# vivansxu/rafiki

Hardware: AMD Instinct MI355X
Metric: images/sec aggregate over concurrent VGG-small 32x32x3 HPO trials (1 trial/GPU) (higher is better)
Workload: dtype fp32; 1 GPU; model=VGG-small 32x32x3 (8 conv3x3+BN+ReLU, 4 maxpool, FC512, FC10), global_batch=256, per_trial_batch=256, parallelism=single trial, 1 GPU, optimizer=SGD nesterov momentum + wd (fused flat-arena kernel), hipgraph=True

## Files before the change

### csrc/kernels/bnf.hip

```cpp
#include "common.h"
#include <algorithm>
#include <cstdint>

namespace {

RK_DEV int rk_log2_dev(int v) { return (v > 0 && (v & (v - 1)) == 0) ? 31 - __builtin_clz(v) : -1; }

RK_DEV int idiv(int a, int d, int log2d) { return log2d >= 0 ? a >> log2d : a / d; }

RK_DEV float act_f(float z, int act, float slope) {
  return act == 1 ? fmaxf(z, 0.f) : act == 2 ? (z > 0.f ? z : z * slope) : z;
}
RK_DEV float act_d(float z, int act, float slope) {
  return act == 1 ? (z > 0.f ? 1.f : 0.f) : act == 2 ? (z > 0.f ? 1.f : slope) : 1.f;
}

template <bool POOL>
__global__ __launch_bounds__(256) void bnf_fwd_kernel(const float* __restrict__ y, const double* __restrict__ slots,
                                                      int SL, double count, const float* __restrict__ gamma,
                                                      const float* __restrict__ beta, float eps, float* rmean,
                                                      float* rvar, float mom, const float* __restrict__ scale_in,
                                                      const float* __restrict__ shift_in, float* __restrict__ coeffs,
                                                      float* __restrict__ out, int Nb, int H, int W, int C, int act,
                                                      float slope) {
  extern __shared__ float s_dyn[];
  float* s_sc = s_dyn;
  float* s_sh = s_dyn + C;
  for (int c = threadIdx.x; c < C; c += 256) {
    float sc, sh;
    if (slots) {
      double s = 0.0, ss = 0.0;
      for (int l = 0; l < SL; ++l) {
        s += slots[(long long)l * 2 * C + c];
        ss += slots[(long long)l * 2 * C + C + c];
      }
      const double mean = s / count;
      const double var = fmax(ss / count - mean * mean, 0.0);
      const double rstd = 1.0 / sqrt(var + (double)eps);
      sc = (float)((double)gamma[c] * rstd);
      sh = (float)((double)beta[c] - mean * (double)gamma[c] * rstd);
      if (blockIdx.x == 0) {
        coeffs[c] = (float)mean;
        coeffs[C + c] = (float)rstd;
        coeffs[2 * C + c] = sc;
        coeffs[3 * C + c] = sh;
        if (rmean) {
          rmean[c] = (float)((1.0 - mom) * rmean[c] + mom * mean);
          rvar[c] = (float)((1.0 - mom) * rvar[c] + mom * var * count / fmax(count - 1.0, 1.0));
        }
      }
    } else {
      sc = scale_in[c];
      sh = shift_in[c];
    }
    s_sc[c] = sc;
    s_sh[c] = sh;
  }
  if (!out) return;
  __syncthreads();
  const int G = C >> 2;
  const int Ho = POOL ? H >> 1 : H, Wo = POOL ? W >> 1 : W;
  const int lG = rk_log2_dev(G), lWo = rk_log2_dev(Wo), lHo = rk_log2_dev(Ho);
  const int total = Nb * Ho * Wo * G;
  for (int i = blockIdx.x * 256 + threadIdx.x; i < total; i += gridDim.x * 256) {
    const int pix = idiv(i, G, lG);
// ... 532 lines not shown
```

### csrc/kernels/winograd4.hip

```cpp
#include <type_traits>
#include "common.h"
#include <cstdlib>

namespace {

#include "wino_wt.h"

constexpr int KC = 8;
enum { WF_RELU = 1, WF_BIAS = 2, WF_STATS = 4, WF_LRELU = 8, WF_BNB = 512, WF_BNP = 1024, WF_POOL = 2048 };
constexpr int WF_POOLED = WF_BIAS | WF_RELU | WF_POOL;

typedef __attribute__((ext_vector_type(2))) float f32x2;

struct W4Params {
  const float* x;
  const float* u;
  float* y;
  const float* bias;
  double* stats;
  const float* gate;
  int Nb, H, W, C, N;
  int TW, THW, ntiles, ncb, slotMask, flags;
  unsigned long long xbytes, ubytes, ybytes;
  int bpg;
  long long gx, gu, gy, gbias;
  const float* pro;
};

constexpr unsigned OOB = 0x80000000u;
constexpr int W4_PRO_MAXC = 512;

RK_DEV int swz(int row) { return ((row >> 2) & 3) << 1; }
RK_DEV int swzw(int row) { return (((row >> 2) & 1) << 1) | (((row >> 3) & 1) << 2) | ((row >> 4) & 1); }
RK_DEV int swzp(int row) { return swzw(row) & 6; }

RK_DEV __amdgpu_buffer_rsrc_t rsrc(const float* base, unsigned long long bytes) {
  return __builtin_amdgcn_make_buffer_rsrc(const_cast<float*>(base), (short)0, (int)(unsigned)bytes, 0x00020000);
}

RK_DEV void bt6(float d0, float d1, float d2, float d3, float d4, float d5, float (&t)[6]) {
  t[0] = 4.f * d0 - 5.f * d2 + d4;
// ... 55 lines not shown
  constexpr int NT = 64 * WM * WN;
  constexpr int T = 16 * WM;
  constexpr int BNC = 16 * WN;
  constexpr int IT = T * KC / NT;
  constexpr int UL = P * BNC * 4 / NT;
  constexpr int UNITS = P * BNC * KC / 4;
  constexpr int UBL = (UNITS + NT - 1) / NT;
  constexpr int ULR = UB ? 1 : UL, UBR = UB ? UBL : 1;
  static_assert(IT >= 1 && IT * NT == T * KC && UL * NT == P * BNC * 4, "tile shape");
  static_assert(!UB || (MO == 4 && BNC == 32), "blocked weights: F(4x4), 32-channel output blocks");
  static_assert(!WS || (NS == 2 && UB), "warp-specialised: two stages, blocked weights");
  __shared__ __attribute__((aligned(16))) float Vs[NS][P][T][KC];
  __shared__ __attribute__((aligned(16))) float Us[NS][P][BNC][KC];
  __shared__ float Ps[PRO ? 2 * W4_PRO_MAXC : 1];
  if constexpr (PRO) {
    for (int i = threadIdx.x; i < 2 * p.C; i += (int)blockDim.x)
      Ps[i < p.C ? i : W4_PRO_MAXC + i - p.C] = p.pro[i];
    __syncthreads();
  }
  const int lane = threadIdx.x & 63, wave = threadIdx.x >> 6;
  const bool compute = !WS || wave < WM * WN;
  const int tid = (WS && !compute) ? (int)threadIdx.x - NT : (int)threadIdx.x;
  const int wm = wave % WM, wn = (wave / WM) % WN;
  const int b0 = xcd_remap(blockIdx.x, gridDim.x);
  const int grp = b0 / p.bpg, b = b0 - grp * p.bpg;
  const int cb = b % p.ncb, tb = b / p.ncb;
  const int tbase = tb * T, cbase = cb * BNC;
  const float* const gxp = p.x + grp * p.gx;
  const float* const gup = p.u + grp * p.gu;
  float* const gyp = p.y + grp * p.gy;
  const float* const gbp = p.bias ? p.bias + grp * p.gbias : nullptr;

// ... 875 lines not shown
                                   const long long* meta, void* stream) {
  if (nblocks <= 0) return RK_OK;
  hipLaunchKernelGGL(wt_all_kernel, dim3(nblocks), dim3(256), 0, (hipStream_t)stream, arena, dst, (const int4*)desc,
                     meta);
  RK_LAUNCH_CHECK();
  return RK_OK;
}

namespace {
struct GfwdArgs {
  const float* x; const float* u; float* y; const float* bias; double* stats; int slotMask; const float* gate;
  int Nb, H, W, C, N, flags, groups;
  long long gx, gu, gy, gbias;
  const float* pro;
  void* stream;
};

template <int MO, int WM, int WN, int MINW, int NS = 1, bool UB = false, bool WS = false, bool PRO = false>
int launch_gfwd(const GfwdArgs& a) {
  constexpr int T = 16 * WM, BNC = 16 * WN, P = (MO + 2) * (MO + 2);
  const int Nb = a.Nb, H = a.H, W = a.W, C = a.C, N = a.N, flags = a.flags, groups = a.groups;
  if (Nb <= 0 || H <= 0 || W <= 0 || (H % MO) || (W % MO) || C <= 0 || (C % KC) || N <= 0 || groups <= 0)
    return RK_EBADARG;
  if ((flags & (WF_STATS | WF_BNB | WF_BNP)) && !a.stats) return RK_EBADARG;
  if ((flags & (WF_BNB | WF_BNP)) && (!a.gate || !a.bias)) return RK_EBADARG;
  if ((flags & WF_BIAS) && !a.bias) return RK_EBADARG;
  if (groups > 1 && (flags & (WF_STATS | WF_BNB | WF_BNP))) return RK_EUNSUPPORTED;
  if (PRO != (a.pro != nullptr)) return RK_EBADARG;
  if ((flags & WF_POOL) && (flags != WF_POOLED || PRO || (H & 1) || (W & 1))) return RK_EUNSUPPORTED;
  if (PRO && (groups > 1 || (flags & ~WF_STATS) || C > W4_PRO_MAXC)) return RK_EUNSUPPORTED;
  W4Params p;
  p.x = a.x; p.u = a.u; p.y = a.y; p.bias = a.bias; p.stats = a.stats; p.gate = a.gate;
  p.pro = a.pro;
  p.Nb = Nb; p.H = H; p.W = W; p.C = C; p.N = N;
  p.TW = W / MO;
  p.THW = (H / MO) * (W / MO);
  const long long nt = (long long)Nb * p.THW;
  if (nt >= (1LL << 30)) return RK_EBADARG;
  p.ntiles = (int)nt;
  p.ncb = rk_cdiv(N, BNC);
  p.xbytes = 4ull * Nb * H * W * C;
  p.ubytes = UB ? 4ull * P * rk_cdiv(N, 32) * 32 * C : 4ull * P * N * C;
  p.ybytes = (flags & WF_POOL) ? 4ull * Nb * (H / 2) * (W / 2) * N : 4ull * Nb * H * W * N;
  const unsigned long long gbytes = (flags & WF_BNP) ? 4 * p.ybytes : p.ybytes;
  if (p.xbytes >= 0x7fffffffull || p.ubytes >= 0x7fffffffull || gbytes >= 0x7fffffffull) return RK_EUNSUPPORTED;
  p.slotMask = a.slotMask;
  p.flags = flags;
  p.gx = a.gx; p.gu = a.gu; p.gy = a.gy; p.gbias = a.gbias;
// ... 57 lines not shown

template <int NR>
int gfwd_dispatch(const GfwdRow (&rows)[NR], int variant, const GfwdArgs& a) {
  for (const GfwdRow& r : rows)
    if (r.variant == variant && r.pro == (a.pro != nullptr)) return r.launch(a);
  return a.pro ? RK_EUNSUPPORTED : RK_EBADARG;
}
}

extern "C" int rk_wino4_conv_grp(const float* x, const float* u, float* y, const float* bias, double* stats,
                                 int slotMask, const float* gate, int Nb, int H, int W, int C, int N, int flags,
                                 int variant, int groups, long long gx, long long gu, long long gy, long long gbias,
                                 const float* pro, void* stream) {
  return gfwd_dispatch(W4_ROWS, variant, {x, u, y, bias, stats, slotMask, gate, Nb, H, W, C, N, flags, groups, gx, gu,
                                          gy, gbias, pro, stream});
}

extern "C" int rk_wino2s_conv_grp(const float* x, const float* u, float* y, const float* bias, double* stats,
                                  int slotMask, const float* gate, int Nb, int H, int W, int C, int N, int flags,
                                  int variant, int groups, long long gx, long long gu, long long gy, long long gbias,
                                  void* stream) {
  return gfwd_dispatch(W2S_ROWS, variant, {x, u, y, bias, stats, slotMask, gate, Nb, H, W, C, N, flags, groups, gx,
                                           gu, gy, gbias, nullptr, stream});
}

extern "C" int rk_wino4_wgrad(const float* dy, const float* x, float* out, int Nb, int H, int W, int Co, int Ci,
                              int splits, int accumulate, int variant, const float* xpro, void* stream) {
  if (Nb <= 0 || H <= 0 || W <= 0 || (H & 3) || (W & 3) || Co <= 0 || Ci <= 0 || splits <= 0) return RK_EBADARG;
  if (splits > 1 && accumulate) return RK_EBADARG;
  if (variant < 0 || variant > 2) return RK_EBADARG;
// ... 60 lines not shown
    }
#pragma unroll
    for (int a = 0; a < 6; ++a) {
      float o[6];
      a6(mm[a][0], mm[a][1], mm[a][2], mm[a][3], o);
#pragma unroll
      for (int b = 0; b < 6; ++b) res[a * 6 + b][e] = o[b];
    }
  }
  float* dst = m + t * C + 4 * c4;
  const int ps = T * C;
#pragma unroll
  for (int q = 0; q < 36; ++q) *(f32x4*)(dst + q * ps) = res[q];
}

template <bool PL = false, int VW = 4>
__global__ __launch_bounds__(256) void w4pt_x_kernel(const float* __restrict__ x, void* __restrict__ v, int H,
                                                     int W, int C, int TW, int THW, int total4, int T,
                                                     const float* __restrict__ pro) {
  typedef __attribute__((ext_vector_type(VW))) float fvec;
  typedef __attribute__((ext_vector_type(VW))) __bf16 bvec;
  const int i = blockIdx.x * 256 + threadIdx.x;
  if (i >= total4) return;
  const int CV = C / VW;
  const int cv = i % CV, t = i / CV;
  const int n = t / THW, r = t - n * THW, ty = r / TW;
  const int oy = 4 * ty - 1, ox = 4 * (r - ty * TW) - 1;
  fvec psc, psh;
#pragma unroll
  for (int e = 0; e < VW; ++e) psc[e] = 1.f, psh[e] = 0.f;
  if (pro) {
    psc = *(const fvec*)(pro + VW * cv);
    psh = *(const fvec*)(pro + C + VW * cv);
  }
  fvec d[36];
#pragma unroll
  for (int a = 0; a < 6; ++a)
#pragma unroll
    for (int b = 0; b < 6; ++b) {
      const int yy = oy + a, xx = ox + b;
      const bool in = (unsigned)yy < (unsigned)H && (unsigned)xx < (unsigned)W;
      fvec val;
      if (in) {
        val = *(const fvec*)(x + ((n * H + yy) * W + xx) * C + VW * cv);
      } else {
#pragma unroll
        for (int e = 0; e < VW; ++e) val[e] = 0.f;
      }
      if (pro && in) {
#pragma unroll
        for (int e = 0; e < VW; ++e) val[e] = fmaxf(fmaf(val[e], psc[e], psh[e]), 0.f);
      }
      d[a * 6 + b] = val;
    }
#pragma unroll
  for (int b = 0; b < 6; ++b)
#pragma unroll
    for (int e = 0; e < VW; ++e) {
      float o[6];
      bt6(d[b][e], d[6 + b][e], d[12 + b][e], d[18 + b][e], d[24 + b][e], d[30 + b][e], o);
#pragma unroll
      for (int a = 0; a < 6; ++a) d[a * 6 + b][e] = o[a];
    }
  const int ps = T * C;
// ... 247 lines not shown

}

extern "C" int rk_wino4_pt_transform(const float* dy, const float* x, float* m, float* v, int Nb, int H, int W,
                                     int Co, int Ci, const float* xpro, void* stream) {
  if (Nb <= 0 || H <= 0 || W <= 0 || (H & 3) || (W & 3) || Co <= 0 || Ci <= 0) return RK_EBADARG;
  if ((Co & 3) || (Ci & 3)) return RK_EUNSUPPORTED;
  const int TW = W / 4, THW = (H / 4) * (W / 4);
  const long long T = (long long)Nb * THW;
  if (36 * T * Co >= (1ll << 31) || 36 * T * Ci >= (1ll << 31)) return RK_EUNSUPPORTED;
  const long long ty = T * Co / 4, tx = T * Ci / 4;
  hipLaunchKernelGGL(w4pt_dy_kernel, dim3((unsigned)((ty + 255) / 256)), dim3(256), 0, (hipStream_t)stream, dy, m, H,
                     W, Co, TW, THW, (int)ty, (int)T);
  RK_LAUNCH_CHECK();
  hipLaunchKernelGGL(w4pt_x_kernel<false>, dim3((unsigned)((tx + 255) / 256)), dim3(256), 0, (hipStream_t)stream, x,
                     v, H, W, Ci, TW, THW, (int)tx, (int)T, xpro);
  RK_LAUNCH_CHECK();
  return RK_OK;
}

extern "C" int rk_wino4_pt_output(const float* du, float* out, int Co, int Ci, int accumulate, int nslab,
                                  long long slab, void* stream) {
  if (Co <= 0 || Ci <= 0 || nslab <= 0 || (nslab > 1 && slab < 36ll * Co * Ci)) return RK_EBADARG;
  if ((Ci & 3) || 36ll * Co * Ci >= (1ll << 31)) return RK_EUNSUPPORTED;
  const long long g2 = (long long)Co * Ci / 2;
  hipLaunchKernelGGL(w4pt_out_kernel, dim3((unsigned)((g2 + 255) / 256)), dim3(256), 0, (hipStream_t)stream, du,
                     out, Co, Ci, accumulate, nslab, slab);
  RK_LAUNCH_CHECK();
  return RK_OK;
}

// ... 234 lines not shown
    if (vw == 4)
      hipLaunchKernelGGL(w4pt_conv_outv_kernel<4>, dim3((unsigned)blocksv), dim3(64), 0, (hipStream_t)stream, yt, y,
                         bias, stats, slotMask, gate, Nb, H, W, N, TW, THW, (int)T, flags, nslab, slab, qs, ts, slope);
    else
      hipLaunchKernelGGL(w4pt_conv_outv_kernel<2>, dim3((unsigned)blocksv), dim3(64), 0, (hipStream_t)stream, yt, y,
                         bias, stats, slotMask, gate, Nb, H, W, N, TW, THW, (int)T, flags, nslab, slab, qs, ts, slope);
    RK_LAUNCH_CHECK();
    return RK_OK;
  }
  hipLaunchKernelGGL(w4pt_conv_out_kernel, dim3((unsigned)blocks), dim3(256), 0, (hipStream_t)stream, yt, y, bias,
                     stats, slotMask, gate, Nb, H, W, N, TW, THW, (int)T, flags, nslab, slab, qs, ts, slope);
  RK_LAUNCH_CHECK();
  return RK_OK;
}

extern "C" int rk_wino4_pt_input(const float* x, float* v, int Nb, int H, int W, int C, const float* pro,
                                 void* stream) {
  if (Nb <= 0 || H <= 0 || W <= 0 || (H & 3) || (W & 3) || C <= 0) return RK_EBADARG;
  if (C & 3) return RK_EUNSUPPORTED;
  const int TW = W / 4, THW = (H / 4) * (W / 4);
  const long long T = (long long)Nb * THW;
  if (36 * T * C >= (1ll << 31)) return RK_EUNSUPPORTED;
  const long long tx = T * C / 4;
  hipLaunchKernelGGL(w4pt_x_kernel<false>, dim3((unsigned)((tx + 255) / 256)), dim3(256), 0, (hipStream_t)stream, x,
                     v, H, W, C, TW, THW, (int)tx, (int)T, pro);
  RK_LAUNCH_CHECK();
  return RK_OK;
}

extern "C" int rk_x6p_w4_input(const float* x, void* v, int Nb, int H, int W, int C, const float* pro,
                               void* stream) {
  if (Nb <= 0 || H <= 0 || W <= 0 || (H & 3) || (W & 3) || C <= 0) return RK_EBADARG;
  if (C & 3) return RK_EUNSUPPORTED;
  const int TW = W / 4, THW = (H / 4) * (W / 4);
  const long long T = (long long)Nb * THW;
  if (108 * T * C >= (1ll << 31) || (long long)Nb * H * W * C >= (1ll << 31)) return RK_EUNSUPPORTED;
  static const int vw = [] {
    const char* e = std::getenv("RAFIKI_PT_X_VW");
    return e && std::atoi(e) == 2 ? 2 : 4;
  }();
  const long long tx = T * C / vw;
  if (vw == 4)
    hipLaunchKernelGGL((w4pt_x_kernel<true, 4>), dim3((unsigned)((tx + 255) / 256)), dim3(256), 0,
                       (hipStream_t)stream, x, v, H, W, C, TW, THW, (int)tx, (int)T, pro);
  else
    hipLaunchKernelGGL((w4pt_x_kernel<true, 2>), dim3((unsigned)((tx + 255) / 256)), dim3(256), 0,
                       (hipStream_t)stream, x, v, H, W, C, TW, THW, (int)tx, (int)T, pro);
  RK_LAUNCH_CHECK();
  return RK_OK;
}

extern "C" int rk_x6p_w4_wgrad_transform(const float* dy, const float* x, void* mt, void* vt, int Nb, int H, int W,
                                         int Co, int Ci, void* stream) {
  if (Nb <= 0 || H <= 0 || W <= 0 || (H & 3) || (W & 3) || Co <= 0 || Ci <= 0) return RK_EBADARG;
  if ((Co & 3) || (Ci & 3)) return RK_EUNSUPPORTED;
  const int TW = W / 4, THW = (H / 4) * (W / 4);
  const long long T = (long long)Nb * THW;
  if (108 * T * Co >= (1ll << 31) || 108 * T * Ci >= (1ll << 31)) return RK_EUNSUPPORTED;
  if ((long long)Nb * H * W * (Co > Ci ? Co : Ci) >= (1ll << 31)) return RK_EUNSUPPORTED;
  if (T % 32 == 0 && Co % 8 == 0 && Ci % 8 == 0) {
    hipLaunchKernelGGL(w4pt_planesT_kernel<true>, dim3((unsigned)(T / 32), Co / 8), dim3(64), 0, (hipStream_t)stream,
                       dy, (bf16*)mt, H, W, Co, TW, THW, (int)T);
    RK_LAUNCH_CHECK();
    hipLaunchKernelGGL(w4pt_planesT_kernel<false>, dim3((unsigned)(T / 32), Ci / 8), dim3(64), 0, (hipStream_t)stream,
// ... 14 lines not shown
```

### rafiki_amd/engine/convnet.py

```python
from __future__ import annotations

import math
import os
import warnings
from typing import List, Optional, Sequence

import numpy as np
import torch
import torch.nn.functional as TF

from ..ops import f32 as S
from ..ops import functional as F
from ..ops.graphs import capture as _capture, device_sync as _device_sync
from .flat import FlatAdam, FlatParams, FlatSGD, check_clip_norm, init_const, init_kaiming

VGG_SMALL_CFG = (64, 64, 'M', 128, 128, 'M', 256, 256, 'M', 512, 512, 'M')
DTYPES = ('fp32', 'bf16')


def default_dtype() -> str:
    d = os.environ.get('RAFIKI_DTYPE', 'fp32').lower()
    d = {'float32': 'fp32', 'f32': 'fp32', 'bfloat16': 'bf16'}.get(d, d)
    if d not in DTYPES:
        raise ValueError('RAFIKI_DTYPE must be one of {}'.format(DTYPES))
# ... 361 lines not shown
        nxt = self.blocks[bi + 1]
        return (not pool and nxt[1] == cout and nxt[4] == hw and ww.lazy('u4b', bi + 1) is not None
                and S.bn_on_load_ok(B, hw, hw, cout, nxt[2]))

    def _fwd_bwd_gpu_f32(self, x, labels):
        fl = self.flat
        B = x.shape[0]
        accs = self._bn_accumulators()
        if not self._acc_zeroed_by_prologue:
            self._bn_acc_flat.zero_()
        ww = self._wino_train()
        if ww is not None:
            ww.refresh()
        acts, saved, h = [x], [], x
        pros, hpro = [None], None
        for bi, (name, cin, cout, pool, hw) in enumerate(self.blocks):
            wk = ww.conv_sets(bi) if ww is not None else {}
            if not self.bn:
                c = self._block_coeffs(bi)
                y = S.conv_fwd(h, fl.w(name + '.w'), bias=fl.w(name + '.b'),
                               act=F.ACT_NONE if pool else F.ACT_RELU, **wk)
                h = S.bn_eval(y, c[2], c[3], pool=True, act=F.ACT_RELU) if pool else y
                saved.append((y, c))
                acts.append(h)
                continue
            rm, rv = self.running_stats(bi)
            y = S.conv_fwd(h, fl.w(name + '.w'), stats_acc=accs[bi][0], pro=hpro, **wk)
            if self._bn_on_load(bi, B, ww):
                coeffs = S.bn_finalize(y, accs[bi][0], B * hw * hw, fl.w(name + '.gamma'), fl.w(name + '.beta'),
                                       self.bn_eps, rm, rv, self.bn_momentum)
                h, hpro = y, coeffs
            else:
                h, coeffs = S.bn_fwd(y, accs[bi][0], B * hw * hw, fl.w(name + '.gamma'), fl.w(name + '.beta'),
                                     self.bn_eps, rm, rv, self.bn_momentum, pool=pool, act=F.ACT_RELU)
                hpro = None
            saved.append((y, coeffs))
            acts.append(h)
            pros.append(hpro)
        in_saved = None
        if self.input_bn:
            raw = h.reshape(B, 1, 1, self.feat_dim)
            acc_f, acc_b = accs[-1]
            S.col_stats(raw.view(B, self.feat_dim), acc_f)
            rm, rv = self.running_stats('in')
            h, coeffs = S.bn_fwd(raw, acc_f, B, fl.w('in_bn.gamma'), fl.w('in_bn.beta'), self.bn_eps, rm, rv,
                                 self.bn_momentum, pool=False, act=F.ACT_NONE)
            in_saved = (raw, coeffs)
        feat = h.reshape(B, self.feat_dim)
        if self.feature_dropout > 0.0:
            self._drop(feat, -1, self.feature_dropout, forward=True)
# ... 740 lines not shown
```

### rafiki_amd/ops/_lib.py

```python
from __future__ import annotations

import ctypes as C
import os
import threading
from pathlib import Path

_NATIVE = Path(__file__).resolve().parent.parent / "_native"
KERNEL_LIB = Path(os.environ["RAFIKI_KERNEL_LIB"]) if os.environ.get("RAFIKI_KERNEL_LIB") else \
    _NATIVE / "librafiki_kernels.so"

_lock = threading.Lock()
_lib = None

vp, i32, i64, f32, f64 = C.c_void_p, C.c_int, C.c_longlong, C.c_float, C.c_double
u32p = C.POINTER(C.c_uint)

_SIGS = {
    "rk_igemm": [i32, i32, i32, vp, vp, vp, vp, vp, vp, i32, i32, i32, i32, i32, i32, i32, i32, i32, i32,
                 i32, i32, i64, i32, f32, f32, i64, i64, vp],
    "rk_hconv": [i32, i32, vp, vp, vp, vp, vp, vp, i32, i32, i32, i32, i32, i32, i32, i32, f32, f32, i64, i64, i32,
                 vp],
    "rk_hconv_wgrad": [vp, vp, vp, i32, i32, i32, i32, i32, i32, i64, i64, vp],
    "rk_bn_bwd_reduce_acc": [vp, vp, vp, vp, vp, i32, i32, i32, i32, i32, i32, i32, i32, f32, vp],
    "rk_bn_bwd_apply_acc": [vp, vp, vp, vp, i32, f64, vp, vp, vp, vp, i32, vp, i32, i32, i32, i32, i32, i32, f32, vp],
# ... 94 lines not shown
    "rk_tag_transpose": [vp, vp, i32, i32, i32, vp],
    "rk_tag_add": [vp, vp, vp, i64, vp],
    "rk_softmax_xent_f32s": [vp, i32, vp, i32, i32, i32, vp, vp, i32, vp, vp],
    "rk_head_fwd_bwd": [vp, i32, i32, vp, vp, i32, vp, i32, f32, vp, vp, i32, vp, vp, vp, vp],
    "rk_head_fwd_bwd_soft": [vp, i32, i32, vp, vp, i32, vp, vp, vp, f32, i32, f32, vp, vp, i32, vp, vp, vp, vp],
    "rk_head_dw": [vp, vp, vp, i32, i32, i32, vp, vp, vp, vp],
    "rk_dropout": [vp, i64, i32, f32, C.c_ulonglong, C.c_uint, vp, vp, vp],
    "rk_x6p_gemm": [i32, i32, vp, vp, vp, i32, i32, i32, i32, i32, i32, i64, i64, i64, i64, i64, i32, i32, i32, i64,
                    i64, i64, vp],
    "rk_x6p_split": [vp, vp, i32, i32, i32, i32, i64, vp],
    "rk_x6p_split_t": [vp, vp, i32, i32, i32, i32, i64, vp],
    "rk_x6p_w4_weights": [vp, vp, vp, i32, i32, vp],
    "rk_wino_weights_all": [vp, vp, vp, i32, vp, vp],
    "rk_x6p_w4_input": [vp, vp, i32, i32, i32, i32, vp, vp],
    "rk_x6p_w4_wgrad_transform": [vp, vp, vp, vp, i32, i32, i32, i32, i32, vp],
}

_RESTYPES = {"rk_embedding_bwd_ws": (C.c_longlong, [i32])}


class NativeLibraryError(RuntimeError):
    pass


class KernelError(RuntimeError):
    pass


def lib():
    global _lib
# ... 43 lines not shown
```

### rafiki_amd/ops/autotune.py

```python
from __future__ import annotations

import fcntl
import hashlib
import json
import os
import sys
import threading

import torch

from .graphs import LOCK as _GRAPH_LOCK, capture as _capture

_lock = threading.Lock()
_cache = {}
_loaded = False
_disk_mtime = [None]
stats = {'tuned': 0, 'seconds': 0.0, 'candidates': 0, 'loaded': 0, 'reloads': 0}
_last_note = [0.0]
ENABLED = os.environ.get('RAFIKI_AUTOTUNE', '1') != '0'
REPS = 3
PASSES = 2
SHIPPED_DIR = os.path.join(os.path.dirname(os.path.dirname(os.path.abspath(__file__))), 'tune')
_ident = {}

# ... 25 lines not shown
                    h.update(f.encode())
                    with open(os.path.join(_SRC_DIR, f), 'rb') as fh:
                        h.update(fh.read())
                _ident['lib'] = 's' + h.hexdigest()[:11]
            else:
                from ._lib import loaded_path as lib_path
                with open(lib_path(), 'rb') as f:
                    for chunk in iter(lambda: f.read(1 << 20), b''):
                        h.update(chunk)
                _ident['lib'] = h.hexdigest()[:12]
        except OSError:
            _ident['lib'] = 'nolib'
    return _ident['lib']


_CAND_SWITCHES = ('RAFIKI_X6', 'RAFIKI_PT_MAX_HW', 'RAFIKI_WINOGRAD', 'RAFIKI_WINOGRAD4')


def db_name() -> str:
    tag = ','.join('{}={}'.format(k, os.environ[k]) for k in _CAND_SWITCHES if k in os.environ)
    suffix = '-' + hashlib.sha1(tag.encode()).hexdigest()[:8] if tag else ''
    return '{}-{}{}.json'.format(_arch(), lib_hash(), suffix)


def _path():
    p = os.environ.get('RAFIKI_TUNE_CACHE')
    if p is not None and p.lower() in ('off', '0', 'none', ''):
        return ''
    if p:
        return p
    from ..config import get_config
# ... 195 lines not shown
```

### rafiki_amd/ops/f32.py

```python
from __future__ import annotations

import os
from functools import partial
from typing import NamedTuple, Optional

import torch

from . import _lib, autotune
from .functional import ACT_LRELU, ACT_NONE, ACT_RELU, _check_soft, bn_slots, cdiv, dropout_

KIND_CONV, KIND_WGRAD, KIND_DENSE, KIND_DENSE_DX, KIND_DENSE_DW = 0, 2, 3, 4, 5
F_RELU, F_BIAS, F_STATS, F_GATE, F_ACCUM, F_LRELU, F_BNB, F_BNP = 1, 2, 4, 8, 16, 32, 512, 1024
TILES = [(128, 128), (128, 64), (64, 128), (64, 64), (256, 64), (256, 128), (128, 256), (64, 256),
         (64, 64), (128, 64), (64, 128)]
_NST3 = (0, 1, 2, 3, 4, 7)
_FEW_WAVE = (8, 9, 10)
NUM_CU = 256
X6 = 16
USE_X6 = os.environ.get('RAFIKI_X6', '1') != '0'


def tile_dims(t: int):
    return TILES[t & 15]

# ... 196 lines not shown
    return on, [c for f, o in zip(families, on) if o for c in f.cfgs]


def _sets_key(sets, on):
    w2, w4, w4b, pt, ptx = on
    return (('lazy' if callable(sets[0]) else w2, 'lazy' if callable(sets[1]) else w4, pt,
             'lazy' if callable(sets[2]) else ptx) + (('b', 'lazy' if callable(sets[3]) else True),) * w4b)


def _run_route(r, x, sets, out, cfg, epi):
    u = sets[r.weights]
    r.kernel(x, u() if callable(u) else u, out=out, **SLOTS[r.slots](r, cfg), **epi)


def conv_fwd(x: torch.Tensor, w: torch.Tensor, *, taps: int = 9, stats_acc=None, bias=None, act=ACT_NONE,
             slope=0.2, out=None, wino=None, wino4=None, wino4p=None, wino4b=None, pro=None):
    _check(x, 'conv_fwd x')
    Nb, H, W, Cin = x.shape
    Cout = w.shape[0]
    M, K = Nb * H * W, taps * Cin
    assert w.numel() == Cout * K, (w.shape, taps, Cin)
    if out is None:
        out = torch.empty((Nb, H, W, Cout), device=x.device, dtype=torch.float32)
    flags = _act_flags(bias, act) | (F_STATS if stats_acc is not None else 0)
    sets = (wino, wino4, wino4p, wino4b)
    epi = dict(bias=bias, stats=stats_acc, relu=act == ACT_RELU)
    need = 0
    if act == ACT_LRELU:
        need, epi['lrelu'] = E_LRELU if stats_acc is None else E_DIRECT, slope
    if pro is not None:
        assert bias is None and act == ACT_NONE and pro.shape == (4, Cin)
# ... 1 lines not shown
    else:
        cands = _cands(M, Cout, splittable=stats_acc is None and Cout % 4 == 0, K=K, big=Cin % 32 == 0)
    on, fused = _offered(CONV_FAMILIES, sets, taps, H, W, Cin, Cout, need)
    cands += fused
    if not cands:
        raise ValueError('conv_fwd(pro=...): no normalise-on-load kernel for this shape (see bn_on_load_ok)')

    def run(cfg):
        r = CONV_ROUTES.get(cfg[0])
        if r is not None:
            _run_route(r, x, sets, out, cfg, epi)
            return
        _gemm(cfg, lambda dst, ldc, **kw: sgemm(KIND_CONV, x, w, dst, M, Cout, K, Cin, K, ldc, H=H, W=W, C=Cin,
                                                taps=taps, **kw),
              out, M, Cout, stats=stats_acc, bias=bias, act=act, slope=slope)
    cfg = _pick(('sf', M, Cout, K, H, W, Cin, taps, flags) + _sets_key(sets, on)
                + (('pro',) if pro is not None else ()), cands, run)
    if stats_acc is not None and autotune.can_tune():
        stats_acc.zero_()
    run(cfg)
    return out


def conv_dgrad(dy: torch.Tensor, wt, *, taps: int = 9, out=None, gate=None, bnb=None, bnp=None,
               wino=None, wino4=None, cin=None, wino4p=None, wino4b=None):
    _check(dy, 'conv_dgrad dy')
    Nb, H, W, Cout = dy.shape
    Cin = cin if callable(wt) else wt.shape[0]
    M, K = Nb * H * W, taps * Cout
    assert callable(wt) or wt.numel() == Cin * K
    if out is None:
        out = torch.empty((Nb, H, W, Cin), device=dy.device, dtype=torch.float32)
# ... 139 lines not shown

def _wino_epilogue(out, bias, stats, relu, bnb, bnp):
    flags = (WF_BIAS if bias is not None else 0) | (WF_RELU if relu else 0) | (WF_STATS if stats is not None else 0)
    gate = None
    if bnb is not None or bnp is not None:
        flags, bias, stats, gate = _bn_bwd_epilogue(out, bnb, bnp)
    if stats is not None:
        assert stats.dtype == torch.float64 and stats.is_contiguous() and stats.shape[-1] == out.shape[-1]
    return flags, bias, stats, gate


def _pro(pro):
    return None if pro is None else _p(pro[2])


def _fused_conv(name, variant, x, u, out, oshape, *, bias=None, stats=None, relu=False, bnb=None, bnp=None,
                pool=False, grp=(1, 0, 0, 0, 0), tail=()):
    Nb, H, W, C = x.shape[-4:]
    if out is None:
        out = torch.empty(oshape, device=x.device, dtype=torch.float32)
    assert out.shape == oshape and out.is_contiguous()
    flags, bias, stats, gate = _wino_epilogue(out, bias, stats, relu, bnb, bnp)
    _lib.call(name, _p(x), _p(u), _p(out), _p(bias), _p(stats), _slots_flags(stats), _p(gate), Nb, H, W, C, oshape[-1],
              flags | (WF_POOL if pool else 0), int(variant), *grp, *tail, _s())
    return out


def _grp_conv(name, variant, P, x, u, out, bias, relu, pool, tail=()):
    G, _, N, C = u.shape
    shared = x.dim() == 4
# ... 39 lines not shown


def wino4_ut(w: torch.Tensor) -> torch.Tensor:
    return wino_set('ut4', w)


def wino4b_numel(N: int, C: int) -> int:
    return 36 * cdiv(N, 32) * 32 * C


def wino4b_u(w: torch.Tensor, dgrad: bool = False) -> torch.Tensor:
    return wino_set('ut4b' if dgrad else 'u4b', w)


def wino4_conv(x: torch.Tensor, u: torch.Tensor, *, out=None, bias=None, stats=None, relu=False, bnb=None, bnp=None,
               variant=0, n_out=None, pro=None):
    _check(x, 'wino4_conv x')
    Nb, H, W, C = x.shape
    if variant >= 3:
        N = int(out.shape[-1] if n_out is None else n_out)
        assert u.dim() == 1 and u.numel() == wino4b_numel(N, C) and u.is_contiguous(), (u.shape, N, C)
    else:
        N = u.shape[1]
        assert u.shape == (36, N, C) and u.is_contiguous(), (u.shape, x.shape)
    if pro is not None:
        assert variant >= 3 and bias is None and not relu and bnb is None and bnp is None
        assert pro.shape == (4, C) and pro.is_contiguous()
    return _fused_conv("rk_wino4_conv_grp", variant, x, u, out, (Nb, H, W, N), bias=bias, stats=stats, relu=relu,
                       bnb=bnb, bnp=bnp, tail=(_pro(pro),))


PT_MAX_HW = int(os.environ.get('RAFIKI_PT_MAX_HW', '32' if USE_X6 else '8'))


def wino4_pt_ok(H, W, C, N):
    return (WINO and WINO4 and H % 4 == 0 and W % 4 == 0 and H <= PT_MAX_HW and W <= PT_MAX_HW and C % 4 == 0
            and C >= 32
            and N >= 32)


def _pt_cfgs(route_id):
    return tuple((route_id, t + x, n) for x in ((0, X6) if USE_X6 else (0,)) for t in (0, 1, 2, 3)
                 for n in ((2, 3) if t in _NST3 else (2,))) + \
        (tuple((route_id, t + X6, 2) for t in _FEW_WAVE) if USE_X6 else ())


def wino4_conv_pt(x: torch.Tensor, u: torch.Tensor, *, out=None, bias=None, stats=None, relu=False, bnb=None,
                  bnp=None, tile=0, nst=2, splits=1, lrelu=None, pro=None):
    _check(x, 'wino4_conv_pt x')
    Nb, H, W, C = x.shape
    planes = u.dtype == torch.bfloat16
    N = u.shape[-2]
    assert u.shape == ((36, 3, N, C) if planes else (36, N, C)) and u.is_contiguous() and H % 4 == 0 and W % 4 == 0, \
        (u.shape, x.shape)
    if out is None:
        out = torch.empty((Nb, H, W, N), device=x.device, dtype=torch.float32)
    assert out.shape == (Nb, H, W, N) and out.is_contiguous()
    flags, bias, stats, gate = _wino_epilogue(out, bias, stats, relu, bnb, bnp)
    if lrelu is not None:
        assert flags in (0, WF_BIAS)
        flags |= WF_LRELU
    T = Nb * (H // 4) * (W // 4)
    if pro is not None:
        assert pro.shape == (4, C) and pro.is_contiguous()
    if planes:
        splits = x6p_splits(C, splits)
        yt = torch.empty((splits, T, 36, N), device=x.device, dtype=torch.float32)
        v = torch.empty((36, 3, T, C), device=x.device, dtype=torch.bfloat16)
        _lib.call("rk_x6p_w4_input", _p(x), _p(v), Nb, H, W, C, _pro(pro), _s())
        x6p_gemm(v, u, yt, T, N, C, groups=36, tile=tile, nst=nst, splits=splits, row_major_groups=True)
    else:
        splits = 1
        yt = torch.empty((36, T, N), device=x.device, dtype=torch.float32)
        v = torch.empty((36, T, C), device=x.device, dtype=torch.float32)
        _lib.call("rk_wino4_pt_input", _p(x), _p(v), Nb, H, W, C, _pro(pro), _s())
        sgemm_grp(KIND_DENSE, v, u, yt, T, N, C, C, C, N, 36, T * C, N * C, T * N, tile=tile, nst=nst)
    _lib.call("rk_wino4_pt_conv_out", _p(yt), _p(out), _p(bias), _p(stats), _slots_flags(stats), _p(gate),
              Nb, H, W, N, flags, splits, 36 * T * N, int(planes), float(0.0 if lrelu is None else lrelu), _s())
    return out


def wino4_conv_grp(x, u, *, out=None, bias=None, relu=False, variant=0, pool=False):
    assert not pool or (bias is not None and relu)
    return _grp_conv("rk_wino4_conv_grp", variant, 36, x, u, out, bias, relu, pool, tail=(None,))


def _wino4_wgrad_cands(Nb, H, W, Cout, Cin):
    if not (WINO and WINO4 and H % 4 == 0 and W % 4 == 0 and Cin >= 8 and Cout >= 16):
        return []
    nt = Nb * (H // 4) * (W // 4)
# ... 886 lines not shown
```

Baseline: 135,500 images/s.

## Fuse BN finalize into next conv's prologue to drop separate kernel launch

Instead of launching a separate bn_finalize kernel between conv layers, the BN statistics reduction (mean, rstd, scale, shift, running stats) is computed in the prologue of the next Winograd conv or input-transform kernel, and block 0 writes the coefficients. This removes one small kernel launch and its dependency gap per BN layer. In exchange, every block of the consumer kernel redundantly reduces the slot statistics in fp64, which adds prologue latency. An environment switch, on by default, controls it and it is added to the autotune key.

```diff
diff --git a/csrc/kernels/bn_fin.h b/csrc/kernels/bn_fin.h
--- /dev/null
+++ b/csrc/kernels/bn_fin.h
@@ -0,0 +1,44 @@
+#pragma once
+#include "common.h"
+
+struct BnFin {
+  const double* slots;
+  int SL;
+  double count;
+  const float* gamma;
+  const float* beta;
+  float eps;
+  float* rmean;
+  float* rvar;
+  float mom;
+  float* coeffs;
+};
+
+RK_DEV void bn_fin_channel(const double* __restrict__ slots, int SL, double count, const float* __restrict__ gamma,
+                           const float* __restrict__ beta, float eps, float* rmean, float* rvar, float mom,
+                           float* __restrict__ coeffs, int C, int c, bool write, float& sc, float& sh) {
+  double s = 0.0, ss = 0.0;
+  for (int l = 0; l < SL; ++l) {
+    s += slots[(long long)l * 2 * C + c];
+    ss += slots[(long long)l * 2 * C + C + c];
+  }
+  const double mean = s / count;
+  const double var = fmax(ss / count - mean * mean, 0.0);
+  const double rstd = 1.0 / sqrt(var + (double)eps);
+  sc = (float)((double)gamma[c] * rstd);
+  sh = (float)((double)beta[c] - mean * (double)gamma[c] * rstd);
+  if (write) {
+    coeffs[c] = (float)mean;
+    coeffs[C + c] = (float)rstd;
+    coeffs[2 * C + c] = sc;
+    coeffs[3 * C + c] = sh;
+    if (rmean) {
+      rmean[c] = (float)((1.0 - mom) * rmean[c] + mom * mean);
+      rvar[c] = (float)((1.0 - mom) * rvar[c] + mom * var * count / fmax(count - 1.0, 1.0));
+    }
+  }
+}
+
+RK_DEV void bn_fin_channel(const BnFin& f, int C, int c, bool write, float& sc, float& sh) {
+  bn_fin_channel(f.slots, f.SL, f.count, f.gamma, f.beta, f.eps, f.rmean, f.rvar, f.mom, f.coeffs, C, c, write, sc, sh);
+}
diff --git a/csrc/kernels/bnf.hip b/csrc/kernels/bnf.hip
--- a/csrc/kernels/bnf.hip
+++ b/csrc/kernels/bnf.hip
@@ -1,3 +1,4 @@
+#include "bn_fin.h"
 #include "common.h"
 #include <algorithm>
 #include <cstdint>
@@ -29,26 +30,7 @@
   for (int c = threadIdx.x; c < C; c += 256) {
     float sc, sh;
     if (slots) {
-      double s = 0.0, ss = 0.0;
-      for (int l = 0; l < SL; ++l) {
-        s += slots[(long long)l * 2 * C + c];
-        ss += slots[(long long)l * 2 * C + C + c];
-      }
-      const double mean = s / count;
-      const double var = fmax(ss / count - mean * mean, 0.0);
-      const double rstd = 1.0 / sqrt(var + (double)eps);
-      sc = (float)((double)gamma[c] * rstd);
-      sh = (float)((double)beta[c] - mean * (double)gamma[c] * rstd);
-      if (blockIdx.x == 0) {
-        coeffs[c] = (float)mean;
-        coeffs[C + c] = (float)rstd;
-        coeffs[2 * C + c] = sc;
-        coeffs[3 * C + c] = sh;
-        if (rmean) {
-          rmean[c] = (float)((1.0 - mom) * rmean[c] + mom * mean);
-          rvar[c] = (float)((1.0 - mom) * rvar[c] + mom * var * count / fmax(count - 1.0, 1.0));
-        }
-      }
+      bn_fin_channel(slots, SL, count, gamma, beta, eps, rmean, rvar, mom, coeffs, C, c, blockIdx.x == 0, sc, sh);
     } else {
       sc = scale_in[c];
       sh = shift_in[c];
diff --git a/csrc/kernels/winograd4.hip b/csrc/kernels/winograd4.hip
--- a/csrc/kernels/winograd4.hip
+++ b/csrc/kernels/winograd4.hip
@@ -1,4 +1,5 @@
 #include <type_traits>
+#include "bn_fin.h"
 #include "common.h"
 #include <cstdlib>
 
@@ -25,6 +26,7 @@
   int bpg;
   long long gx, gu, gy, gbias;
   const float* pro;
+  BnFin fin;
 };
 
 constexpr unsigned OOB = 0x80000000u;
@@ -110,8 +112,13 @@
   __shared__ __attribute__((aligned(16))) float Us[NS][P][BNC][KC];
   __shared__ float Ps[PRO ? 2 * W4_PRO_MAXC : 1];
   if constexpr (PRO) {
-    for (int i = threadIdx.x; i < 2 * p.C; i += (int)blockDim.x)
-      Ps[i < p.C ? i : W4_PRO_MAXC + i - p.C] = p.pro[i];
+    if (p.fin.slots) {
+      for (int c = threadIdx.x; c < p.C; c += (int)blockDim.x)
+        bn_fin_channel(p.fin, p.C, c, blockIdx.x == 0, Ps[c], Ps[W4_PRO_MAXC + c]);
+    } else {
+      for (int i = threadIdx.x; i < 2 * p.C; i += (int)blockDim.x)
+        Ps[i < p.C ? i : W4_PRO_MAXC + i - p.C] = p.pro[i];
+    }
     __syncthreads();
   }
   const int lane = threadIdx.x & 63, wave = threadIdx.x >> 6;
@@ -1017,6 +1024,7 @@
   long long gx, gu, gy, gbias;
   const float* pro;
   void* stream;
+  BnFin fin = {};
 };
 
 template <int MO, int WM, int WN, int MINW, int NS = 1, bool UB = false, bool WS = false, bool PRO = false>
@@ -1030,11 +1038,15 @@
   if ((flags & WF_BIAS) && !a.bias) return RK_EBADARG;
   if (groups > 1 && (flags & (WF_STATS | WF_BNB | WF_BNP))) return RK_EUNSUPPORTED;
   if (PRO != (a.pro != nullptr)) return RK_EBADARG;
+  if (a.fin.slots && (a.fin.SL <= 0 || !a.fin.gamma || !a.fin.beta || !a.fin.coeffs || a.pro != a.fin.coeffs + 2 * C ||
+                      !a.fin.rmean != !a.fin.rvar))
+    return RK_EBADARG;
   if ((flags & WF_POOL) && (flags != WF_POOLED || PRO || (H & 1) || (W & 1))) return RK_EUNSUPPORTED;
   if (PRO && (groups > 1 || (flags & ~WF_STATS) || C > W4_PRO_MAXC)) return RK_EUNSUPPORTED;
   W4Params p;
   p.x = a.x; p.u = a.u; p.y = a.y; p.bias = a.bias; p.stats = a.stats; p.gate = a.gate;
   p.pro = a.pro;
+  p.fin = a.fin;
   p.Nb = Nb; p.H = H; p.W = W; p.C = C; p.N = N;
   p.TW = W / MO;
   p.THW = (H / MO) * (W / MO);
@@ -1122,6 +1134,17 @@
                                  const float* pro, void* stream) {
   return gfwd_dispatch(W4_ROWS, variant, {x, u, y, bias, stats, slotMask, gate, Nb, H, W, C, N, flags, groups, gx, gu,
                                           gy, gbias, pro, stream});
+}
+
+extern "C" int rk_wino4_conv_fin(const float* x, const float* u, float* y, double* stats, int slotMask, int Nb, int H,
+                                 int W, int C, int N, int flags, int variant, const double* slots, int SL,
+                                 double count, const float* gamma, const float* beta, float eps, float* rmean,
+                                 float* rvar, float mom, float* coeffs, void* stream) {
+  if (!slots || !coeffs) return RK_EBADARG;
+  GfwdArgs a = {x, u, y, nullptr, stats, slotMask, nullptr, Nb, H, W, C, N, flags, 1, 0, 0, 0, 0, coeffs + 2 * C,
+                stream};
+  a.fin = {slots, SL, count, gamma, beta, eps, rmean, rvar, mom, coeffs};
+  return gfwd_dispatch(W4_ROWS, variant, a);
 }
 
 extern "C" int rk_wino2s_conv_grp(const float* x, const float* u, float* y, const float* bias, double* stats,
@@ -1212,12 +1235,19 @@
   for (int q = 0; q < 36; ++q) *(f32x4*)(dst + q * ps) = res[q];
 }
 
-template <bool PL = false, int VW = 4>
+constexpr int W4PT_FIN_MAXC = 1024;
+template <bool PL = false, int VW = 4, bool FIN = false>
 __global__ __launch_bounds__(256) void w4pt_x_kernel(const float* __restrict__ x, void* __restrict__ v, int H,
                                                      int W, int C, int TW, int THW, int total4, int T,
-                                                     const float* __restrict__ pro) {
+                                                     const float* __restrict__ pro, const BnFin fin) {
   typedef __attribute__((ext_vector_type(VW))) float fvec;
   typedef __attribute__((ext_vector_type(VW))) __bf16 bvec;
+  __shared__ __attribute__((aligned(16))) float Fs[FIN ? 2 * W4PT_FIN_MAXC : 4];
+  if constexpr (FIN) {
+    for (int c = threadIdx.x; c < C; c += 256)
+      bn_fin_channel(fin, C, c, blockIdx.x == 0, Fs[c], Fs[W4PT_FIN_MAXC + c]);
+    __syncthreads();
+  }
   const int i = blockIdx.x * 256 + threadIdx.x;
   if (i >= total4) return;
   const int CV = C / VW;
@@ -1227,7 +1257,10 @@
   fvec psc, psh;
 #pragma unroll
   for (int e = 0; e < VW; ++e) psc[e] = 1.f, psh[e] = 0.f;
-  if (pro) {
+  if constexpr (FIN) {
+    psc = *(const fvec*)(Fs + VW * cv);
+    psh = *(const fvec*)(Fs + W4PT_FIN_MAXC + VW * cv);
+  } else if (pro) {
     psc = *(const fvec*)(pro + VW * cv);
     psh = *(const fvec*)(pro + C + VW * cv);
   }
@@ -1245,7 +1278,7 @@
 #pragma unroll
         for (int e = 0; e < VW; ++e) val[e] = 0.f;
       }
-      if (pro && in) {
+      if ((FIN || pro) && in) {
 #pragma unroll
         for (int e = 0; e < VW; ++e) val[e] = fmaxf(fmaf(val[e], psc[e], psh[e]), 0.f);
       }
@@ -1523,7 +1556,7 @@
                      W, Co, TW, THW, (int)ty, (int)T);
   RK_LAUNCH_CHECK();
   hipLaunchKernelGGL(w4pt_x_kernel<false>, dim3((unsigned)((tx + 255) / 256)), dim3(256), 0, (hipStream_t)stream, x,
-                     v, H, W, Ci, TW, THW, (int)tx, (int)T, xpro);
+                     v, H, W, Ci, TW, THW, (int)tx, (int)T, xpro, BnFin{});
   RK_LAUNCH_CHECK();
   return RK_OK;
 }
@@ -1788,23 +1821,33 @@
   return RK_OK;
 }
 
-extern "C" int rk_wino4_pt_input(const float* x, float* v, int Nb, int H, int W, int C, const float* pro,
-                                 void* stream) {
-  if (Nb <= 0 || H <= 0 || W <= 0 || (H & 3) || (W & 3) || C <= 0) return RK_EBADARG;
+namespace {
+bool w4pt_fin_ok(const BnFin& f, int C) {
+  return !f.slots || (f.SL > 0 && f.gamma && f.beta && f.coeffs && C <= W4PT_FIN_MAXC && !f.rmean == !f.rvar);
+}
+
+int launch_pt_input(const float* x, float* v, int Nb, int H, int W, int C, const float* pro, const BnFin& fin,
+                    void* stream) {
+  if (Nb <= 0 || H <= 0 || W <= 0 || (H & 3) || (W & 3) || C <= 0 || !w4pt_fin_ok(fin, C)) return RK_EBADARG;
   if (C & 3) return RK_EUNSUPPORTED;
   const int TW = W / 4, THW = (H / 4) * (W / 4);
   const long long T = (long long)Nb * THW;
   if (36 * T * C >= (1ll << 31)) return RK_EUNSUPPORTED;
   const long long tx = T * C / 4;
-  hipLaunchKernelGGL(w4pt_x_kernel<false>, dim3((unsigned)((tx + 255) / 256)), dim3(256), 0, (hipStream_t)stream, x,
-                     v, H, W, C, TW, THW, (int)tx, (int)T, pro);
+  const dim3 grid((unsigned)((tx + 255) / 256));
+  if (fin.slots)
+    hipLaunchKernelGGL((w4pt_x_kernel<false, 4, true>), grid, dim3(256), 0, (hipStream_t)stream, x, v, H, W, C, TW,
+                       THW, (int)tx, (int)T, pro, fin);
+  else
+    hipLaunchKernelGGL(w4pt_x_kernel<false>, grid, dim3(256), 0, (hipStream_t)stream, x, v, H, W, C, TW, THW,
+                       (int)tx, (int)T, pro, fin);
   RK_LAUNCH_CHECK();
   return RK_OK;
 }
 
-extern "C" int rk_x6p_w4_input(const float* x, void* v, int Nb, int H, int W, int C, const float* pro,
-                               void* stream) {
-  if (Nb <= 0 || H <= 0 || W <= 0 || (H & 3) || (W & 3) || C <= 0) return RK_EBADARG;
+int launch_x6p_input(const float* x, void* v, int Nb, int H, int W, int C, const float* pro, const BnFin& fin,
+                     void* stream) {
+  if (Nb <= 0 || H <= 0 || W <= 0 || (H & 3) || (W & 3) || C <= 0 || !w4pt_fin_ok(fin, C)) return RK_EBADARG;
   if (C & 3) return RK_EUNSUPPORTED;
   const int TW = W / 4, THW = (H / 4) * (W / 4);
   const long long T = (long long)Nb * THW;
@@ -1814,14 +1857,43 @@
     return e && std::atoi(e) == 2 ? 2 : 4;
   }();
   const long long tx = T * C / vw;
-  if (vw == 4)
-    hipLaunchKernelGGL((w4pt_x_kernel<true, 4>), dim3((unsigned)((tx + 255) / 256)), dim3(256), 0,
-                       (hipStream_t)stream, x, v, H, W, C, TW, THW, (int)tx, (int)T, pro);
+  const dim3 grid((unsigned)((tx + 255) / 256));
+  const hipStream_t st = (hipStream_t)stream;
+  if (vw == 4 && fin.slots)
+    hipLaunchKernelGGL((w4pt_x_kernel<true, 4, true>), grid, dim3(256), 0, st, x, v, H, W, C, TW, THW, (int)tx, (int)T,
+                       pro, fin);
+  else if (vw == 4)
+    hipLaunchKernelGGL((w4pt_x_kernel<true, 4>), grid, dim3(256), 0, st, x, v, H, W, C, TW, THW, (int)tx, (int)T, pro,
+                       fin);
+  else if (fin.slots)
+    hipLaunchKernelGGL((w4pt_x_kernel<true, 2, true>), grid, dim3(256), 0, st, x, v, H, W, C, TW, THW, (int)tx, (int)T,
+                       pro, fin);
   else
-    hipLaunchKernelGGL((w4pt_x_kernel<true, 2>), dim3((unsigned)((tx + 255) / 256)), dim3(256), 0,
-                       (hipStream_t)stream, x, v, H, W, C, TW, THW, (int)tx, (int)T, pro);
+    hipLaunchKernelGGL((w4pt_x_kernel<true, 2>), grid, dim3(256), 0, st, x, v, H, W, C, TW, THW, (int)tx, (int)T, pro,
+                       fin);
   RK_LAUNCH_CHECK();
   return RK_OK;
+}
+}
+
+extern "C" int rk_wino4_pt_input(const float* x, float* v, int Nb, int H, int W, int C, const float* pro,
+                                 void* stream) {
+  return launch_pt_input(x, v, Nb, H, W, C, pro, BnFin{}, stream);
+}
+
+extern "C" int rk_x6p_w4_input(const float* x, void* v, int Nb, int H, int W, int C, const float* pro,
+                               void* stream) {
+  return launch_x6p_input(x, v, Nb, H, W, C, pro, BnFin{}, stream);
+}
+
+extern "C" int rk_wino4_pt_input_fin(const float* x, void* v, int Nb, int H, int W, int C, int planes,
+                                     const double* slots, int SL, double count, const float* gamma,
+                                     const float* beta, float eps, float* rmean, float* rvar, float mom,
+                                     float* coeffs, void* stream) {
+  if (!slots || !coeffs) return RK_EBADARG;
+  const BnFin fin = {slots, SL, count, gamma, beta, eps, rmean, rvar, mom, coeffs};
+  return planes ? launch_x6p_input(x, v, Nb, H, W, C, nullptr, fin, stream)
+                : launch_pt_input(x, (float*)v, Nb, H, W, C, nullptr, fin, stream);
 }
 
 extern "C" int rk_x6p_w4_wgrad_transform(const float* dy, const float* x, void* mt, void* vt, int Nb, int H, int W,
diff --git a/rafiki_amd/engine/convnet.py b/rafiki_amd/engine/convnet.py
--- a/rafiki_amd/engine/convnet.py
+++ b/rafiki_amd/engine/convnet.py
@@ -399,6 +399,7 @@
             ww.refresh()
         acts, saved, h = [x], [], x
         pros, hpro = [None], None
+        hfin = None
         for bi, (name, cin, cout, pool, hw) in enumerate(self.blocks):
             wk = ww.conv_sets(bi) if ww is not None else {}
             if not self.bn:
@@ -410,15 +411,19 @@
                 acts.append(h)
                 continue
             rm, rv = self.running_stats(bi)
-            y = S.conv_fwd(h, fl.w(name + '.w'), stats_acc=accs[bi][0], pro=hpro, **wk)
+            y = S.conv_fwd(h, fl.w(name + '.w'), stats_acc=accs[bi][0], pro=hpro, fin=hfin, **wk)
             if self._bn_on_load(bi, B, ww):
-                coeffs = S.bn_finalize(y, accs[bi][0], B * hw * hw, fl.w(name + '.gamma'), fl.w(name + '.beta'),
-                                       self.bn_eps, rm, rv, self.bn_momentum)
+                fin = S.BnFin(accs[bi][0], B * hw * hw, fl.w(name + '.gamma'), fl.w(name + '.beta'), self.bn_eps,
+                              rm, rv, self.bn_momentum)
+                coeffs = torch.empty((4, cout), device=y.device, dtype=torch.float32)
+                hfin = fin if S.BN_FIN_FUSED else None
+                if hfin is None:
+                    fin.run(y, coeffs)
                 h, hpro = y, coeffs
             else:
                 h, coeffs = S.bn_fwd(y, accs[bi][0], B * hw * hw, fl.w(name + '.gamma'), fl.w(name + '.beta'),
                                      self.bn_eps, rm, rv, self.bn_momentum, pool=pool, act=F.ACT_RELU)
-                hpro = None
+                hpro = hfin = None
             saved.append((y, coeffs))
             acts.append(h)
             pros.append(hpro)
diff --git a/rafiki_amd/ops/_lib.py b/rafiki_amd/ops/_lib.py
--- a/rafiki_amd/ops/_lib.py
+++ b/rafiki_amd/ops/_lib.py
@@ -132,6 +132,9 @@
     "rk_wino_weights_all": [vp, vp, vp, i32, vp, vp],
     "rk_x6p_w4_input": [vp, vp, i32, i32, i32, i32, vp, vp],
     "rk_x6p_w4_wgrad_transform": [vp, vp, vp, vp, i32, i32, i32, i32, i32, vp],
+    "rk_wino4_conv_fin": [vp, vp, vp, vp, i32, i32, i32, i32, i32, i32, i32, i32, vp, i32, f64, vp, vp, f32, vp, vp,
+                          f32, vp, vp],
+    "rk_wino4_pt_input_fin": [vp, vp, i32, i32, i32, i32, i32, vp, i32, f64, vp, vp, f32, vp, vp, f32, vp, vp],
 }
 
 _RESTYPES = {"rk_embedding_bwd_ws": (C.c_longlong, [i32])}
diff --git a/rafiki_amd/ops/autotune.py b/rafiki_amd/ops/autotune.py
--- a/rafiki_amd/ops/autotune.py
+++ b/rafiki_amd/ops/autotune.py
@@ -63,7 +63,7 @@
     return _ident['lib']
 
 
-_CAND_SWITCHES = ('RAFIKI_X6', 'RAFIKI_PT_MAX_HW', 'RAFIKI_WINOGRAD', 'RAFIKI_WINOGRAD4')
+_CAND_SWITCHES = ('RAFIKI_X6', 'RAFIKI_PT_MAX_HW', 'RAFIKI_WINOGRAD', 'RAFIKI_WINOGRAD4', 'RAFIKI_BN_FIN_FUSED')
 
 
 def db_name() -> str:
diff --git a/rafiki_amd/ops/f32.py b/rafiki_amd/ops/f32.py
--- a/rafiki_amd/ops/f32.py
+++ b/rafiki_amd/ops/f32.py
@@ -234,7 +234,7 @@
 
 
 def conv_fwd(x: torch.Tensor, w: torch.Tensor, *, taps: int = 9, stats_acc=None, bias=None, act=ACT_NONE,
-             slope=0.2, out=None, wino=None, wino4=None, wino4p=None, wino4b=None, pro=None):
+             slope=0.2, out=None, wino=None, wino4=None, wino4p=None, wino4b=None, pro=None, fin=None):
     _check(x, 'conv_fwd x')
     Nb, H, W, Cin = x.shape
     Cout = w.shape[0]
@@ -266,8 +266,14 @@
         _gemm(cfg, lambda dst, ldc, **kw: sgemm(KIND_CONV, x, w, dst, M, Cout, K, Cin, K, ldc, H=H, W=W, C=Cin,
                                                 taps=taps, **kw),
               out, M, Cout, stats=stats_acc, bias=bias, act=act, slope=slope)
-    cfg = _pick(('sf', M, Cout, K, H, W, Cin, taps, flags) + _sets_key(sets, on)
-                + (('pro',) if pro is not None else ()), cands, run)
+    key = ('sf', M, Cout, K, H, W, Cin, taps, flags) + _sets_key(sets, on) + (('pro',) if pro is not None else ())
+    if fin is not None:
+        assert pro is not None
+        if autotune.ENABLED and autotune.can_tune() and not autotune._valid(autotune.lookup(key), cands):
+            fin.run(x, pro)
+        else:
+            epi['fin'] = fin
+    cfg = _pick(key, cands, run)
     if stats_acc is not None and autotune.can_tune():
         stats_acc.zero_()
     run(cfg)
@@ -437,6 +443,31 @@
     return None if pro is None else _p(pro[2])
 
 
+BN_FIN_FUSED = os.environ.get('RAFIKI_BN_FIN_FUSED', '1') != '0'
+
+
+class BnFin(NamedTuple):
+    acc: torch.Tensor
+    count: float
+    gamma: torch.Tensor
+    beta: torch.Tensor
+    eps: float
+    running_mean: Optional[torch.Tensor] = None
+    running_var: Optional[torch.Tensor] = None
+    momentum: float = 0.1
+
+    def args(self, coeffs):
+        C = coeffs.shape[1]
+        assert self.acc.dtype == torch.float64 and self.acc.is_contiguous() and self.acc.shape[1:] == (2, C)
+        assert coeffs.shape == (4, C) and coeffs.is_contiguous() and self.gamma.numel() == C and self.beta.numel() == C
+        return (_p(self.acc), self.acc.shape[0], float(self.count), _p(self.gamma), _p(self.beta), float(self.eps),
+                _p(self.running_mean), _p(self.running_var), float(self.momentum), _p(coeffs))
+
+    def run(self, y, coeffs):
+        return bn_finalize(y, self.acc, self.count, self.gamma, self.beta, self.eps, self.running_mean,
+                           self.running_var, self.momentum, coeffs=coeffs)
+
+
 def _fused_conv(name, variant, x, u, out, oshape, *, bias=None, stats=None, relu=False, bnb=None, bnp=None,
                 pool=False, grp=(1, 0, 0, 0, 0), tail=()):
     Nb, H, W, C = x.shape[-4:]
@@ -506,7 +537,7 @@
 
 
 def wino4_conv(x: torch.Tensor, u: torch.Tensor, *, out=None, bias=None, stats=None, relu=False, bnb=None, bnp=None,
-               variant=0, n_out=None, pro=None):
+               variant=0, n_out=None, pro=None, fin=None):
     _check(x, 'wino4_conv x')
     Nb, H, W, C = x.shape
     if variant >= 3:
@@ -518,6 +549,14 @@
     if pro is not None:
         assert variant >= 3 and bias is None and not relu and bnb is None and bnp is None
         assert pro.shape == (4, C) and pro.is_contiguous()
+    if fin is not None:
+        if out is None:
+            out = torch.empty((Nb, H, W, N), device=x.device, dtype=torch.float32)
+        assert pro is not None and out.shape == (Nb, H, W, N) and out.is_contiguous()
+        flags, _, stats, _ = _wino_epilogue(out, None, stats, False, None, None)
+        _lib.call("rk_wino4_conv_fin", _p(x), _p(u), _p(out), _p(stats), _slots_flags(stats), Nb, H, W, C, N, flags,
+                  int(variant), *fin.args(pro), _s())
+        return out
     return _fused_conv("rk_wino4_conv_grp", variant, x, u, out, (Nb, H, W, N), bias=bias, stats=stats, relu=relu,
                        bnb=bnb, bnp=bnp, tail=(_pro(pro),))
 
@@ -538,7 +577,7 @@
 
 
 def wino4_conv_pt(x: torch.Tensor, u: torch.Tensor, *, out=None, bias=None, stats=None, relu=False, bnb=None,
-                  bnp=None, tile=0, nst=2, splits=1, lrelu=None, pro=None):
+                  bnp=None, tile=0, nst=2, splits=1, lrelu=None, pro=None, fin=None):
     _check(x, 'wino4_conv_pt x')
     Nb, H, W, C = x.shape
     planes = u.dtype == torch.bfloat16
@@ -555,17 +594,24 @@
     T = Nb * (H // 4) * (W // 4)
     if pro is not None:
         assert pro.shape == (4, C) and pro.is_contiguous()
+    assert fin is None or pro is not None
+
+    def transform(entry, v):
+        if fin is not None:
+            _lib.call("rk_wino4_pt_input_fin", _p(x), _p(v), Nb, H, W, C, int(planes), *fin.args(pro), _s())
+        else:
+            _lib.call(entry, _p(x), _p(v), Nb, H, W, C, _pro(pro), _s())
     if planes:
         splits = x6p_splits(C, splits)
         yt = torch.empty((splits, T, 36, N), device=x.device, dtype=torch.float32)
         v = torch.empty((36, 3, T, C), device=x.device, dtype=torch.bfloat16)
-        _lib.call("rk_x6p_w4_input", _p(x), _p(v), Nb, H, W, C, _pro(pro), _s())
+        transform("rk_x6p_w4_input", v)
         x6p_gemm(v, u, yt, T, N, C, groups=36, tile=tile, nst=nst, splits=splits, row_major_groups=True)
     else:
         splits = 1
         yt = torch.empty((36, T, N), device=x.device, dtype=torch.float32)
         v = torch.empty((36, T, C), device=x.device, dtype=torch.float32)
-        _lib.call("rk_wino4_pt_input", _p(x), _p(v), Nb, H, W, C, _pro(pro), _s())
+        transform("rk_wino4_pt_input", v)
         sgemm_grp(KIND_DENSE, v, u, yt, T, N, C, C, C, N, 36, T * C, N * C, T * N, tile=tile, nst=nst)
     _lib.call("rk_wino4_pt_conv_out", _p(yt), _p(out), _p(bias), _p(stats), _slots_flags(stats), _p(gate),
               Nb, H, W, N, flags, splits, 36 * T * N, int(planes), float(0.0 if lrelu is None else lrelu), _s())
```

Measured after the change: 135,900 images/s (median of 6 runs). No clear change (+0.3%).
